# arkworks-rs/algebra

Hardware: AMD Instinct MI355X
Metric: G1 scalar-muls/sec (MSM, 2^24) (higher is better)
Workload: dtype u32

## Files before the change

### algebra_amd/_lib.py

```python
import ctypes as C
import os

_HERE = os.path.dirname(os.path.abspath(__file__))
LIB_PATH = os.environ.get("ARK_HIP_LIB") or os.path.join(_HERE, "libark_hip.so")

u64p = C.POINTER(C.c_uint64)


class ArkHipError(RuntimeError):
    def __init__(self, code, what):
        super().__init__("%s failed with code %d" % (what, code))
        self.code = code


class Radix2DomainStruct(C.Structure):
    _fields_ = [
        ("size", C.c_uint64),
        ("log_size_of_group", C.c_uint32),
        ("_pad", C.c_uint32),
        ("size_as_field_element", C.c_uint64 * 4),
        ("size_inv", C.c_uint64 * 4),
        ("group_gen", C.c_uint64 * 4),
        ("group_gen_inv", C.c_uint64 * 4),
        ("offset", C.c_uint64 * 4),
# ... 129 lines not shown
    "ark_hip_test_basefield_op": (C.c_int, [C.c_int, C.c_int, C.c_void_p, C.c_void_p, C.c_void_p, C.c_size_t]),
    "ark_hip_test_host_basefield_op": (C.c_int, [C.c_int, C.c_int, C.c_void_p, C.c_void_p, C.c_void_p, C.c_size_t]),
    "ark_hip_test_host_sw_check": (C.c_int, [C.c_int, C.c_void_p, C.c_size_t, C.c_int, C.c_int, C.c_void_p]),
    "ark_hip_test_host_sw_decompress": (C.c_int, [C.c_int, C.c_void_p, C.c_size_t, C.c_int, C.c_int, C.c_void_p, C.c_void_p]),
    "ark_hip_test_host_sw_compress": (C.c_int, [C.c_int, C.c_void_p, C.c_size_t, C.c_void_p]),
    "ark_hip_test_host_sw_mul": (C.c_int, [C.c_int, C.c_void_p, C.c_int, C.c_void_p, C.c_size_t, C.c_int, C.c_int, C.c_size_t, C.c_void_p]),
    "ark_hip_test_host_sw_add": (C.c_int, [C.c_int, C.c_void_p, C.c_void_p, C.c_int, C.c_size_t, C.c_void_p]),
    "ark_hip_test_host_sw_fold": (C.c_int, [C.c_int, C.c_void_p, C.c_void_p, C.c_int, C.c_void_p, C.c_void_p, C.c_int, C.c_int, C.c_size_t,
                                            C.c_void_p]),
    "ark_hip_test_coord_sqrt": (C.c_int, [C.c_int, C.c_void_p, C.c_void_p, C.c_void_p, C.c_size_t]),
    "ark_hip_test_host_coord_sqrt": (C.c_int, [C.c_int, C.c_void_p, C.c_void_p, C.c_void_p, C.c_size_t]),
    "ark_hip_test_point_op": (C.c_int, [C.c_int, C.c_int, C.c_void_p, C.c_void_p, C.c_void_p, C.c_size_t]),
    "ark_hip_test_msm_sharded_emulated": (C.c_int, [C.c_int, C.c_int, C.POINTER(C.c_void_p), C.POINTER(C.c_void_p),
                                                    C.POINTER(C.c_size_t), C.c_int, C.c_void_p, C.POINTER(C.c_int)]),
    "ark_hip_test_base_hash": (C.c_int, [C.c_void_p, C.c_size_t, C.POINTER(C.c_uint64)]),
    "ark_hip_test_lazy_raw_op": (C.c_int, [C.c_int, C.c_int, C.c_int, C.c_int, C.c_void_p, C.c_void_p, C.c_size_t]),
    "ark_hip_test_lazy_acc_op": (C.c_int, [C.c_int, C.c_int, C.c_void_p, C.c_void_p, C.c_void_p, C.c_size_t]),
    "ark_hip_test_relaxed_raw_op": (C.c_int, [C.c_int, C.c_int, C.c_void_p, C.c_void_p, C.c_size_t]),
    "ark_hip_test_relaxed_acc_op": (C.c_int, [C.c_int, C.c_int, C.c_void_p, C.c_void_p, C.c_void_p, C.c_size_t]),
    "ark_hip_test_msm_host_fold": (C.c_int, [C.c_int, C.c_void_p, C.c_int, C.c_int, C.c_int, C.c_void_p, C.c_void_p]),
    "ark_hip_test_msm_reduce_geometry": (C.c_int, [C.c_int, C.c_int, C.c_int, C.c_int, C.c_int, C.c_size_t, C.POINTER(C.c_uint32)]),
    "ark_hip_test_msm_sort_geometry": (C.c_int, [C.c_int, C.c_size_t, C.c_int, C.c_int, C.c_int, C.c_int, C.POINTER(C.c_int32),
                                                 C.POINTER(C.c_uint64)]),
    "ark_hip_test_msm_sort_stages": (C.c_int, [C.c_int, C.c_void_p, C.c_int, C.c_size_t, C.c_int, C.c_int, C.c_int,
                                               C.POINTER(C.c_int32), C.POINTER(C.c_uint64), C.POINTER(C.c_void_p),
                                               C.POINTER(C.c_size_t)]),
    "ark_hip_test_msm_pieces": (C.c_int, [C.c_int, C.c_void_p, C.c_void_p, C.c_int, C.c_size_t, C.c_int, C.POINTER(C.c_size_t), C.c_int,
                                          C.POINTER(C.c_int32), C.POINTER(C.c_uint64), C.c_void_p, C.c_size_t, C.c_void_p, C.c_size_t,
                                          C.c_void_p]),
    "ark_hip_test_msm_host_fold_l0": (C.c_int, [C.c_int, C.c_void_p, C.c_int, C.c_int, C.c_int, C.c_void_p, C.c_void_p]),
}
TEST_LIB_PATH = os.path.join(_HERE, "libark_hip_test.so")

_lib = None
_test_lib = None


def lib():
    global _lib
    if _lib is None:
        if not os.path.exists(LIB_PATH):
            raise ImportError(
                "algebra_amd: %s not found -- the HIP extension is not built and there is no CPU fallback "
                "(run `make -C algebra_amd/csrc -j8` or __graft_entry__.build())" % LIB_PATH)
        try:
            import torch
# ... 40 lines not shown
```

### algebra_amd/csrc/msm.cuh

```cuda
#pragma once
#include <hip/hip_runtime.h>
#include <stdio.h>
#include <stdlib.h>
#include <vector>
#include <mutex>
#include <atomic>
#include "hostpool.hpp"
#include <math.h>
#include "curves.cuh"
#include "ec28.cuh"
#include "lazyk.cuh"
#include "msm_sort.cuh"
#include "msm_plan.hpp"

namespace arkhip {

#define ARK_HIP_TRY(expr)                                                                          \
  do {                                                                                             \
    hipError_t _e = (expr);                                                                        \
    if (_e != hipSuccess) {                                                                        \
      fprintf(stderr, "ark_hip: %s failed: %s (%s:%d)\n", #expr, hipGetErrorString(_e), __FILE__, __LINE__); \
      return -(int)_e - 1000;                                                                      \
    }                                                                                              \
  } while (0)
// ... 161 lines not shown
template <class SP>
void msm_sample_widths_host(const void* h_scalars, size_t n, int mont, MsmWidths* out) {
  typedef Fp<SP> S;
  *out = MsmWidths{};
  out->max_bits = (u32)SP::BITS;
  if (n == 0) return;
  const size_t stride = n > 1024 ? n / 1024 : 1;
  size_t seen = 0;
  u32 cnt[MSM_WIDTH_CLASSES] = {0};
  for (size_t i = 0; i < n; i += stride) {
    u32 v[S::N + 1];
    (void)msm_scalar_magnitude<SP>((const u32*)h_scalars, (u32)i, mont, v, nullptr);
    u32 b = 0;
    for (int k = 0; k < S::N; k++)
      if (v[k]) b = 32u * (u32)k + 32u - (u32)__builtin_clz(v[k]);
    int cls = 0;
    for (int k = 1; k < MSM_WIDTH_CLASSES; k++) cls += b > (u32)MSM_WIDTH_TOP[k - 1] ? 1 : 0;
    cnt[cls]++;
    seen++;
  }
  for (int k = 0; k < MSM_WIDTH_CLASSES; k++) out->count[k] = (u32)((double)cnt[k] * (double)n / (double)seen);
}

template <class SP>
__global__ void __launch_bounds__(256) msm_digits_kernel(const u32* __restrict__ scalars, u32 n, int mont, int c,
                                                         int W, int narrow, u32* __restrict__ keys,
                                                         u32* __restrict__ err) {
  u32 i = blockIdx.x * blockDim.x + threadIdx.x;
  if (i >= n) return;
  typedef Fp<SP> S;
  u32 v[S::N + 1];
  const u32 flip = msm_scalar_magnitude<SP>(scalars, i, mont, v, err);
  u32 carry = 0;
  for (int w = 0; w < W; w++) {
    const int cw = msm_window_width(w, c, W, narrow);
    const u32 mask = (1u << cw) - 1u;
    const u32 half = 1u << (cw - 1);
    u32 raw = (v[0] & mask) + carry;
#pragma unroll
    for (int k = 0; k < S::N; k++) v[k] = (v[k] >> cw) | (v[k + 1] << (32 - cw));
    u32 key = KEY_NONE;
    if (w < W - 1) {
      carry = raw >= half ? 1u : 0u;
    } else {
      carry = 0;
    }
    int d = (int)raw - (int)(carry << cw);
    if (d != 0) {
      u32 mag = d < 0 ? (u32)(-d) : (u32)d;
      if (mag > half) {
        atomicOr(err, 1u);
        mag = half;
      }
      u32 sign = (d < 0 ? 0x80000000u : 0u) ^ flip;
      key = sign | (mag - 1);
    }
    keys[(size_t)w * n + i] = key;
  }
}

template <int BYTES>
__global__ void __launch_bounds__(256) msm_digits_small_kernel(const unsigned char* __restrict__ scalars, u32 n, int c, int W,
                                                               int narrow, u64 vmask, u32* __restrict__ keys) {
  u32 i = blockIdx.x * blockDim.x + threadIdx.x;
  if (i >= n) return;
  u64 v;
  if constexpr (BYTES == 1) v = scalars[i];
  else if constexpr (BYTES == 2) v = ((const unsigned short*)scalars)[i];
  else if constexpr (BYTES == 4) v = ((const u32*)scalars)[i];
  else v = ((const u64*)scalars)[i];
  v &= vmask;
  u32 carry = 0;
  for (int w = 0; w < W; w++) {
    const int cw = msm_window_width(w, c, W, narrow);
    const u32 mask = (1u << cw) - 1u;
    const u32 half = 1u << (cw - 1);
    const u32 raw = ((u32)v & mask) + carry;
    v >>= cw;
    carry = (w < W - 1 && raw >= half) ? 1u : 0u;
    const int d = (int)raw - (int)(carry << cw);
    u32 key = KEY_NONE;
// ... 927 lines not shown
    const bool fail =
        (compacted && (cscal.ensure(n * 32) || cidx.ensure(n * 4))) ||
        keys.ensure(W * n * 4) || sorted.ensure(W * n * 4) || part.ensure(W * n * 8) ||
        thist.ensure(sg.nthist * 4) || toff.ensure((sg.nthist + 2) * 4) ||
        offsets.ensure((pl.nb + 2) * 4) || sums.ensure(2 * sg.nsums * 4) ||
        order.ensure(nbk * 4) || ohist.ensure((sg.nohist + ORDER_BINS) * 4) || ooff.ensure((sg.nohist + ORDER_BINS + 2) * 4) ||
        (own_buckets && buckets.ensure(nbk * B)) ||
        lvlS[0].ensure(rg.m * Wr * B) || lvlA[0].ensure(rg.m * Wr * B) || lvlS[1].ensure(rg.npart * B) ||
        (rg.nchunks > 1 && lvlA[1].ensure(rg.npairs * B)) || (rg.two_digit && lvlA[1].ensure(Wr * rg.nsum2 * B)) ||
        hctr.ensure(64) || hlist.ensure((hg.max_heavy + 1) * sizeof(HeavyEntry)) || hitems.ensure((hg.max_items + 1) * 8) ||
        hpart.ensure((hg.max_items + 1) * B) || (pl.shared && hfinal.ensure(hg.max_heavy * B)) ||
        (sg.big_on && big.ensure(2 * sg.big_region * 4)) || (run_parts > 1 && parts.ensure(2 * (size_t)run_parts * pl.nb * B));
    return fail ? -3 : 0;
  }
  int launch_resources(bool need_side) {
    if (need_side) {
      if (!side) ARK_HIP_TRY(hipStreamCreateWithFlags(&side, hipStreamNonBlocking));
      for (auto& e : grp_ev)
        if (!e) ARK_HIP_TRY(hipEventCreateWithFlags(&e, hipEventDisableTiming));
    }
    if (!attr_set) {
      ARK_HIP_TRY(hipFuncSetAttribute((const void*)msm_part_scatter_kernel, hipFuncAttributeMaxDynamicSharedMemorySize,
                                      (int)PART_SCATTER_LDS_MAX));
      ARK_HIP_TRY(hipFuncSetAttribute((const void*)msm_part_finish_kernel, hipFuncAttributeMaxDynamicSharedMemorySize,
                                      160 * 1024 - 64));
      attr_set = true;
    }
    return 0;
  }
  void release() {
    if (probe_host) (void)hipHostFree(probe_host);
    probe_host = nullptr;
    hctr.release(); hlist.release(); hitems.release(); hpart.release(); hfinal.release();
    nzcnt.release(); cscal.release(); cidx.release();
    keys.release(); part.release(); thist.release(); toff.release(); sorted.release();
    offsets.release(); sums.release();
    order.release(); ohist.release(); ooff.release(); probe.release(); big.release(); parts.release();
    buckets.release();
    if (side) { (void)hipStreamSynchronize(side); (void)hipStreamDestroy(side); side = nullptr; }
    for (auto& e : grp_ev) { if (e) (void)hipEventDestroy(e); e = nullptr; }
    for (int i = 0; i < 2; i++) { lvlS[i].release(); lvlA[i].release(); }
    for (auto& j : jobs) {
      if (j.pinned) (void)hipHostFree(j.pinned);
      j.pinned = nullptr;
      j.pinned_cap = 0;
      if (j.done) (void)hipEventDestroy(j.done);
      if (j.acc_done) (void)hipEventDestroy(j.acc_done);
// ... 99 lines not shown
template <class C>
struct MsmCall {
  typedef XYZZ<typename C::F> Pt;
  MsmWorkspace& ws;
  MsmJob& job;
  hipStream_t stream;
  bool timing;
  const void* d_points;
  size_t wstride;
  const void* d_scalars;
  size_t n;
  int scalars_mont;
  const MsmPiece* piece;
  MsmPlan pl;
  MsmSortGeom sg;
  MsmReduceGeom rg;
  MsmHeavyGeom hg;
  int ngroups;
  bool heavy_side, lazy, compacted;
  u32 run_parts;
  int split_level;
  char* d_buckets;
  int accum;

  struct Group {
    int w0, Wg;
    size_t slot0, nslots, nbk_g;
    u32 *keys, *sorted, *offsets, *thist, *toff, *order, *sums, *ohist, *ooff, *hctr;
    u32* big;
    u32* big_count;
    uint2* part;
    HeavyEntry* hlist;
    uint2* hitems;
    char *hpart, *buckets, *parts;
    size_t max_heavy;
  } grp[2];

  void make_groups() {
    const int W = pl.W, Bbits = pl.c - 1;
    const size_t nbk = pl.nbuckets();
    const int W0 = ngroups == 2 ? (W + 1) / 2 : W;
    for (int g = 0; g < ngroups; g++) {
      Group& G = grp[g];
      G.w0 = g == 0 ? 0 : W0;
      G.Wg = g == 0 ? W0 : W - W0;
      G.slot0 = (size_t)G.w0 << Bbits;
// ... 23 lines not shown
      G.parts = run_parts > 1 ? (char*)ws.parts.p + (size_t)g * run_parts * pl.nb * Pt::BYTES : nullptr;
    }
  }

  void compact(const void* d_scalars_all, size_t n_all, const MsmProbe& pr) {
    u32* const cnt = (u32*)ws.nzcnt.p;
    u32* const off = cnt + pr.nz_blocks + 1;
    scan_exclusive(cnt, pr.nz_blocks, nullptr, off, stream);
    hipLaunchKernelGGL((msm_compact_scalars_kernel<typename C::S>), dim3(pr.nz_blocks), dim3(1024), 0, stream,
                       (const u32*)d_scalars_all, (u32)n_all, scalars_mont, pr.nz_chunk, (const u32*)off, (u32*)ws.hctr.p + 3,
                       (u32*)ws.cscal.p, (u32*)ws.cidx.p, (u32)n);
  }

  void digits(int sbytes, int sbits) {
    const int c = pl.c, W = pl.W;
    u32* const keys = (u32*)ws.keys.p;
    const u32 nblk = (u32)((n + 255) / 256);
    if (sbytes) {
      const u64 vmask = sbits >= 64 ? ~0ull : ((1ull << sbits) - 1ull);
      const unsigned char* sp = (const unsigned char*)d_scalars;
      const auto kernel = sbytes == 1 ? msm_digits_small_kernel<1> : sbytes == 2 ? msm_digits_small_kernel<2>
                          : sbytes == 4 ? msm_digits_small_kernel<4> : msm_digits_small_kernel<8>;
      hipLaunchKernelGGL(kernel, dim3(nblk), dim3(256), 0, stream, sp, (u32)n, c, W, pl.narrow, vmask, keys);
    } else {
      hipLaunchKernelGGL((msm_digits_kernel<typename C::S>), dim3(nblk), dim3(256), 0, stream, (const u32*)d_scalars,
                         (u32)n, scalars_mont, c, W, pl.narrow, keys, (u32*)ws.hctr.p + 3);
    }
  }

  int sort_group(const Group& G, hipStream_t st, bool mark) {
    const int HB = sg.HB, LB = sg.LB;
    const u32 ntiles = sg.ntiles;
    const size_t mwin = (size_t)1 << (pl.c - 1);
    const u32 nsuper_g = (u32)G.Wg << HB;
    const size_t nthist_g = (size_t)nsuper_g * ntiles;
    hipLaunchKernelGGL(msm_part_hist_kernel, dim3(ntiles, G.Wg), dim3(256), (size_t)4 << HB, st, G.keys, (u32)n, HB, LB,
                       ntiles, sg.tile, G.thist);
    scan_exclusive(G.thist, nthist_g, G.sums, G.toff, st);
    if (mark && timing) ARK_HIP_TRY(hipEventRecord(job.ev[2], st));
    hipLaunchKernelGGL(msm_part_scatter_kernel, dim3(ntiles, G.Wg), dim3(1024), sg.lds_a, st, G.keys, (u32)n, HB, LB, ntiles,
                       sg.tile, G.toff, G.part, compacted ? (const u32*)ws.cidx.p : (const u32*)nullptr);
    hipLaunchKernelGGL(msm_part_finish_kernel, dim3(nsuper_g), dim3(1024), sg.lds_b, st, G.part, G.toff, ntiles, LB, nsuper_g,
                       sg.stage_cap, sg.big_on ? PART_BIG : 0u, G.big_count, G.big, G.offsets, G.sorted);
    if (sg.big_on) {
      u32* const bigcnt = G.big + nsuper_g;
      u32* const cursor = bigcnt + G.nslots;
      hipLaunchKernelGGL(msm_part_big_hist_kernel, dim3(PART_BIG_SLICES, PART_BIG_GRID_Y), dim3(1024), (size_t)4 << LB, st,
                         G.part, G.toff, ntiles, LB, G.big_count, G.big, bigcnt);
      hipLaunchKernelGGL(msm_part_big_place_kernel, dim3(PART_BIG_SLICES, PART_BIG_GRID_Y), dim3(1024),
                         ((size_t)8 << LB) + 4096, st, G.part, G.toff, ntiles, LB, G.big_count, G.big, bigcnt, cursor, G.offsets,
                         G.sorted);
    }
    int shift = 0;
    while ((hg.mean_load >> shift) >= 64) shift++;
    const u32 noblk_g = (u32)((G.nbk_g + ORDER_TILE - 1) / ORDER_TILE);
    const int wsum = pl.shared ? pl.W : 1;
    hipLaunchKernelGGL(msm_order_hist_kernel, dim3(noblk_g), dim3(256), 0, st, G.offsets, G.nbk_g, shift, noblk_g, wsum, mwin,
                       G.ohist);
    scan_exclusive(G.ohist, (size_t)noblk_g * ORDER_BINS, G.sums, G.ooff, st);
    hipLaunchKernelGGL(msm_order_scatter_kernel, dim3(noblk_g), dim3(256), 0, st, G.offsets, G.nbk_g, shift, noblk_g, wsum, mwin,
                       G.ooff, G.order);
    return 0;
  }

  int front(const void* d_scalars_all, size_t n_all, const MsmProbe& pr, int sbytes, int sbits) {
    if (timing) ARK_HIP_TRY(hipEventRecord(job.ev[0], stream));
// ... 113 lines not shown
      job.short_job = (double)n * (double)pl.W <= 6.0e6;
      job.Q = rg.Q;
      job.d_sums = d_sums;
    }
    job.busy = true;
    return 0;
  }
};

template <class C>
struct MsmSetup {
  MsmProbe pr;
  MsmPlan pl;
  size_t n_all, n;
  bool compacted;
  MsmSortGeom sg;
  MsmReduceGeom rg;
  MsmHeavyGeom hg;
  bool lazy;
  u32 run_parts;
  int ngroups;
  bool heavy_side;
  int split_level;
  MsmCall<C> call(MsmWorkspace& ws, MsmJob& job, hipStream_t stream, bool timing, const void* d_points, size_t wstride,
                  const void* d_scalars, int scalars_mont, const MsmPiece* piece, char* d_buckets) const {
    MsmCall<C> c{ws, job, stream, timing, d_points, wstride, compacted ? ws.cscal.p : d_scalars, n, scalars_mont, piece,
                 pl, sg, rg, hg, ngroups, heavy_side, lazy, compacted, run_parts, split_level,
                 d_buckets, (piece && !piece->first) ? 1 : 0};
    c.make_groups();
    return c;
  }
};
template <class C>
int msm_setup(MsmWorkspace& ws, const void* d_scalars, size_t n, int scalars_mont, hipStream_t stream, int sbytes, int sbits,
              const MsmPlan*& prepared, size_t& wstride, const MsmPiece* piece, const MsmKnobs& knobs, MsmSetup<C>& su) {
  MsmProbe& pr = su.pr;
  if (!sbytes && !piece && n >= ((size_t)1 << 19))
    if (int rc = msm_probe_widths<C>(ws, d_scalars, n, scalars_mont, stream, knobs, prepared, wstride, pr)) return rc;
  const MsmPlan pl = prepared ? *prepared
                     : piece  ? *piece->plan
                     : pr.have_widths ? msm_plan_for_widths(C::ID, n, pr.widths, knobs)
                                      : msm_default_plan(C::ID, n, sbytes ? sbits + 1 : C::S::BITS, false, nullptr, knobs);
  const size_t n_all = n, zeros = pr.widths.count[0];
  const bool compacted = pr.measured_exact && knobs.compact && zeros * 4 >= n && zeros < n && zeros * (size_t)pl.W >= 3 * n;
  if (compacted) n = n_all - zeros;
  if ((size_t)n * (size_t)pl.W >= (1ull << 32)) return -2;
  if (prepared && (wstride < n || (size_t)pl.W * wstride >= (1ull << 31))) return -2;

  su.pl = pl;
  su.n_all = n_all;
  su.n = n;
  su.compacted = compacted;
  su.sg = msm_sort_geometry(n, pl, knobs);
  if (su.sg.lds_a > PART_SCATTER_LDS_MAX) return -2;
  su.rg = msm_reduce_geometry(pl, C::FA::LANES, C::S::BITS, C::FA::LANES == 1 ? msm_resident_lanes<C>() : 0, knobs);
  su.hg = msm_heavy_geometry(n, pl, knobs);
  su.lazy = knobs.lazy;
  su.run_parts = (su.lazy && !piece && !pl.shared) ? msm_run_parts(n, pl, pr.have_widths ? &pr.widths : nullptr, knobs) : 1u;
  su.ngroups = msm_window_groups(n, pl, piece != nullptr, knobs);
  su.heavy_side = knobs.heavy_side && su.ngroups == 1 && !piece && n >= ((size_t)1 << 20);
  su.split_level = knobs.split_level;
  return 0;
}

template <class C>
int msm_enqueue(MsmWorkspace& ws, const void* d_points, size_t wstride, const MsmPlan* prepared, const void* d_scalars,
                size_t n, int scalars_mont, hipStream_t stream, bool timing, int sbytes = 0, int sbits = 0,
                const MsmPiece* piece = nullptr, const MsmKnobs* knobs_in = nullptr) {
  typedef XYZZ<typename C::F> Pt;
  std::lock_guard<std::mutex> lock(ws.mu);
  int slot = -1;
  for (int i = 0; i < MSM_JOBS; i++)
    if (!ws.jobs[i].busy) { slot = i; break; }
  if (slot < 0) return -6;
  MsmJob& job = ws.jobs[slot];
  job.empty = (n == 0);
  job.timing = false;
  job.no_result = false;
  if (piece && (prepared || n == 0)) return -1;
  if (n == 0) {
    job.busy = true;
    return slot;
  }
  if (n >= (1ull << 31)) return -2;
// ... 313 lines not shown
```

### algebra_amd/csrc/msm_plan.hpp

```cpp
#pragma once
#include <math.h>
#include <stddef.h>
#include <stdint.h>
#include <stdio.h>
#include <stdlib.h>
#include "params.hpp"

#if defined(__HIP__)
#define ARK_PLAN_HD __host__ __device__ __forceinline__
#else
#define ARK_PLAN_HD inline
#endif

namespace arkhip {
typedef uint32_t u32;

struct MsmKnobs {
  bool lazy = true;
  bool probe = true;
  bool compact = true;
  bool heavy_side = true;
  bool big_slices = true;
  bool plan_debug = false;
  int groups = 0;
  int split_level = -1;
  size_t parts_lanes = 262144;
  int c = 0;
  int c_prepared = 0;
  int l0 = 0;
  int stage2 = -1;
  int chunk = 0;
  int heavy = 0;
  int hb = -1;
  int tile = 0;
  int run_parts = 0;
};

inline MsmKnobs msm_knobs() {
  const auto first_char = [](const char* name) { const char* e = getenv(name); return e ? e[0] : '\0'; };
  const auto number = [](const char* name, long unset) { const char* e = getenv(name); return e ? atol(e) : unset; };
  const auto within = [](long v, long lo, long hi) { return v >= lo && v <= hi ? (int)v : 0; };
  static const MsmKnobs once = [&] {
    MsmKnobs k;
    k.lazy = first_char("ARK_HIP_MSM_LAZY") != '0';
    k.probe = number("ARK_HIP_MSM_PROBE", 1) != 0;
    k.compact = first_char("ARK_HIP_MSM_COMPACT") != '0';
    k.heavy_side = number("ARK_HIP_MSM_HEAVY_SIDE", 1) != 0;
    k.big_slices = number("ARK_HIP_MSM_BIG_SLICES", 1) != 0;
    k.plan_debug = getenv("ARK_HIP_PLAN_DEBUG") != nullptr;
    k.groups = (int)number("ARK_HIP_MSM_GROUPS", 0);
    k.split_level = (int)number("ARK_HIP_MSM_SPLIT_LEVEL", -1);
    k.parts_lanes = (size_t)number("ARK_HIP_MSM_PARTS_LANES", 262144);
    return k;
  }();
  MsmKnobs k = once;
  k.c = within(number("ARK_HIP_MSM_C", 0), 3, 26);
  k.c_prepared = within(number("ARK_HIP_MSM_C_PREPARED", 0), 3, 26);
  k.l0 = within(number("ARK_HIP_MSM_L0", 0), 1, 128);
  const char s2 = first_char("ARK_HIP_MSM_STAGE2");
  k.stage2 = s2 == '0' ? 0 : (s2 == '1' ? 1 : -1);
  const long chunk = number("ARK_HIP_MSM_CHUNK", 0);
  k.chunk = (chunk & (chunk - 1)) == 0 ? within(chunk, 256, 16384) : 0;
  k.heavy = within(number("ARK_HIP_MSM_HEAVY", 0), 64, 0x7fffffff);
  k.hb = (int)number("ARK_HIP_MSM_HB", -1);
  k.tile = (int)number("ARK_HIP_MSM_TILE", 0);
  const long rp = number("ARK_HIP_MSM_RUN_PARTS", 0);
  k.run_parts = (rp & (rp - 1)) == 0 ? within(rp, 1, 8) : 0;
  return k;
}

static constexpr int MSM_WIDTH_CLASSES = 9;
static constexpr int MSM_WIDTH_TOP[MSM_WIDTH_CLASSES] = {0, 1, 8, 16, 32, 64, 128, 192, 256};
struct MsmWidths {
  u32 max_bits;
  u32 count[MSM_WIDTH_CLASSES];
// ... 145 lines not shown
  p.nb = (size_t)p.W << (best_c - 1);
  return p;
}

static inline MsmPlan msm_default_plan(int curve_id, size_t n, int bits, bool shared, const MsmWidths* widths,
                                       const MsmKnobs& knobs = msm_knobs(), bool streamed = false) {
  return msm_make_plan(n, bits, msm_mul_cost(curve_id), shared, widths, !shared && !streamed && knobs.lazy, knobs);
}

static inline MsmPlan msm_plan_for_widths(int curve_id, size_t n, const MsmWidths& w, const MsmKnobs& knobs = msm_knobs()) {
  const int slack = 8, field_bits = msm_scalar_bits(curve_id);
  int bits = field_bits;
  if ((int)w.max_bits + 1 + slack <= field_bits) bits = (w.max_bits ? (int)w.max_bits : 1) + 1;
  return msm_default_plan(curve_id, n, bits, false, &w, knobs);
}

static constexpr int PART_LO_BITS = 10;
static constexpr int PART_LO_BITS_MAX = 12;
static constexpr u32 PART_LDS_WORDS = (160 * 1024 - 64) / 4;
static constexpr int PART_TILE = 8192;
static constexpr int PART_TILE_BIG = 16384;
static constexpr size_t PART_SCATTER_LDS_MAX = 160 * 1024 - 4096 - 64;
static constexpr u32 PART_BIG = 1u << 17;
static constexpr int SCAN_TILE = 2048;
static constexpr int ORDER_TILE = 2048;
static constexpr int ORDER_BINS = 256;

static inline void msm_part_split(size_t n, int B, int* HB, int* LB, const MsmKnobs& knobs) {
  int hb = 0;
  if (B > PART_LO_BITS) {
    hb = B - PART_LO_BITS;
    if (hb > 9) {
      hb = B - PART_LO_BITS_MAX;
      if (hb < 9) hb = 9;
    }
    int lg = 0;
    while (((size_t)1 << lg) < n) lg++;
    if (hb < lg - 15) hb = lg - 15;
    if (hb > B) hb = B;
    const int v = knobs.hb;
    if (v >= 0 && v <= B && B - v <= PART_LO_BITS_MAX) hb = v;
  } else {
    int lg = 0;
    while (((size_t)1 << lg) < n) lg++;
    hb = lg - 15;
    if (hb < 0) hb = 0;
    if (hb > B) hb = B;
  }
  *HB = hb;
  *LB = B - hb;
}
static inline u32 msm_part_stage_cap(int LB) { return PART_LDS_WORDS - 1024u - (1u << LB) - 16u; }
static inline u32 msm_part_tile(int HB, const MsmKnobs& knobs) {
  const bool fits = ((size_t)8 << HB) + (size_t)PART_TILE_BIG * 8 <= PART_SCATTER_LDS_MAX;
  if (knobs.tile == PART_TILE || (knobs.tile == PART_TILE_BIG && fits)) return (u32)knobs.tile;
  return (HB >= 11 && fits) ? (u32)PART_TILE_BIG : (u32)PART_TILE;
}

struct MsmSortGeom {
  int HB, LB;
  u32 nsuper;
  u32 tile, ntiles;
  size_t nthist;
  size_t lds_a, lds_b;
  u32 stage_cap;
  bool big_on;
  size_t big_region;
  u32 noblk;
  size_t nohist, nsums;
};
static inline MsmSortGeom msm_sort_geometry(size_t n, const MsmPlan& pl, const MsmKnobs& knobs) {
  MsmSortGeom g;
  msm_part_split(n, pl.c - 1, &g.HB, &g.LB, knobs);
  g.nsuper = (u32)pl.W << g.HB;
  g.tile = msm_part_tile(g.HB, knobs);
  g.ntiles = (u32)((n + g.tile - 1) / g.tile);
  g.nthist = (size_t)g.nsuper * g.ntiles;
  g.lds_a = ((size_t)8 << g.HB) + (size_t)g.tile * 8;
  g.stage_cap = msm_part_stage_cap(g.LB);
  g.lds_b = ((size_t)(1 << g.LB) + 1024 + g.stage_cap) * 4;
  g.big_on = knobs.big_slices && n > (size_t)2 * PART_BIG;
  g.big_region = (size_t)g.nsuper + 2 * pl.nb;
  const u32 ntscan = (u32)((g.nthist + SCAN_TILE - 1) / SCAN_TILE);
  g.noblk = (u32)((pl.nbuckets() + ORDER_TILE - 1) / ORDER_TILE);
  g.nohist = (size_t)g.noblk * ORDER_BINS;
  const u32 noscan = (u32)((g.nohist + SCAN_TILE - 1) / SCAN_TILE);
  g.nsums = (size_t)(ntscan > noscan ? ntscan : noscan) + 2;
  return g;
}

struct MsmReduceGeom {
  u32 red_narrow, red_full;
  u32 L0;
  size_t m, mn;
  int nbits;
  u32 Q;
  bool two_digit;
  u32 d2, rows2;
  size_t nsum2;
  u32 chunk, nchunks;
  size_t npart, npairs;
};
// ... 74 lines not shown

static inline u32 msm_run_parts(size_t n, const MsmPlan& pl, const MsmWidths* widths, const MsmKnobs& knobs) {
  u32 run_parts = 1;
  double expect = (double)n * pl.W;
  if (widths) {
    expect = 0.0;
    for (int k = 1; k < MSM_WIDTH_CLASSES; k++) {
      int need = (MSM_WIDTH_TOP[k] + 1 + pl.c - 1) / pl.c;
      expect += (double)widths->count[k] * (need > pl.W ? pl.W : need);
    }
  }
  const double mean_run = expect / (double)pl.nb;
  while (run_parts < 8 && pl.nb * (size_t)(2 * run_parts) <= knobs.parts_lanes && mean_run >= 32.0 * (2 * run_parts)) run_parts *= 2;
  if (pl.parts) run_parts = pl.parts;
  if (knobs.run_parts) run_parts = (u32)knobs.run_parts;
  return run_parts;
}

static inline int msm_window_groups(size_t n, const MsmPlan& pl, bool piece, const MsmKnobs& knobs) {
  if (pl.shared || piece || pl.W < 6 || n < ((size_t)1 << 19)) return 1;
  return (knobs.groups == 2 || (knobs.groups != 1 && n >= ((size_t)1 << 25))) ? 2 : 1;
}

}
```

### algebra_amd/csrc/msm_sort.cuh

```cuda
#pragma once
#include <hip/hip_runtime.h>
#include <stdlib.h>
#include "fp.cuh"
#include "msm_plan.hpp"

namespace arkhip {

static constexpr u32 PART_KEY_NONE = 0xffffffffu;
static constexpr int PART_MLP = 8;
static constexpr int PART_OUT_MLP = 4;
static constexpr int PART_SCATTER_KEYS = PART_TILE_BIG / 1024;

__host__ __device__ __forceinline__ u32 msm_slot_to_bucket(u32 slot, int HB, int LB) {
  const u32 B = (u32)(HB + LB);
  const u32 w = slot >> B;
  const u32 in = slot & ((1u << B) - 1u);
  const u32 low = in >> LB;
  const u32 high = in & ((1u << LB) - 1u);
  return (w << B) | (high << HB) | low;
}

static __device__ __forceinline__ u32 part_tile_of_block(u32 b, u32 ntiles) {
  const u32 per = ntiles >> 3;
  return b < (per << 3) ? (b & 7u) * per + (b >> 3) : b;
// ... 109 lines not shown
      if (j < total) {
        const u32 bkt = e[b].x & 0x7fffffffu;
        part[dst[b]] = make_uint2((bkt >> HB) | (e[b].x & 0x80000000u), e[b].y);
      }
    }
  }
}

__device__ __forceinline__ u32 lds_inc_leading(u32* cnt, u32 key) {
  const u32 k0 = __builtin_amdgcn_readfirstlane(key);
  const unsigned long long same = __ballot(key == k0);
  u32 pos;
  if (key == k0) {
    const u32 rank = __builtin_amdgcn_mbcnt_hi((u32)(same >> 32), __builtin_amdgcn_mbcnt_lo((u32)same, 0u));
    u32 base = 0;
    if (rank == 0) base = atomicAdd(&cnt[k0], (u32)__popcll(same));
    pos = __builtin_amdgcn_readfirstlane(base) + rank;
  } else {
    pos = atomicAdd(&cnt[key], 1u);
  }
  return pos;
}

static __global__ void __launch_bounds__(1024) msm_part_finish_kernel(const uint2* __restrict__ part,
                                                                      const u32* __restrict__ tile_off, u32 ntiles,
                                                                      int LB, u32 nsuper, u32 stage_cap, u32 big_thresh,
                                                                      u32* __restrict__ big_count, u32* __restrict__ big,
                                                                      u32* __restrict__ offsets,
                                                                      u32* __restrict__ sorted) {
  extern __shared__ u32 part_lds[];
  const u32 nlow = 1u << LB;
  u32* cnt = part_lds;
  u32* wsum = part_lds + nlow;
  u32* stage = wsum + 1024;
  const u32 sb = blockIdx.x;
  const u32 start = tile_off[(size_t)sb * ntiles];
  const u32 end = tile_off[(size_t)(sb + 1) * ntiles];
  if (sb == nsuper - 1 && threadIdx.x == 0) offsets[(size_t)nsuper << LB] = end;
  if (big_thresh && end - start > big_thresh) {
    if (threadIdx.x == 0) big[atomicAdd(big_count, 1u)] = sb;
    u32* const bigcnt = big + nsuper + ((size_t)sb << LB);
    u32* const cursor = bigcnt + ((size_t)nsuper << LB);
    for (u32 b = threadIdx.x; b < nlow; b += blockDim.x) {
      bigcnt[b] = 0;
      cursor[b] = 0;
    }
    return;
  }
  for (u32 b = threadIdx.x; b < nlow; b += blockDim.x) cnt[b] = 0;
  __syncthreads();
  const u32 lmask = nlow - 1u;
  for (u32 c0 = start; c0 < end; c0 += blockDim.x * PART_MLP) {
    u32 kx[PART_MLP];
#pragma unroll
    for (int b = 0; b < PART_MLP; b++) {
      const u32 j = c0 + (u32)b * blockDim.x + threadIdx.x;
      kx[b] = j < end ? part[j].x : PART_KEY_NONE;
    }
#pragma unroll
    for (int b = 0; b < PART_MLP; b++)
      if (kx[b] != PART_KEY_NONE) lds_inc_leading(cnt, kx[b] & lmask);
  }
  __syncthreads();
  const u32 per = nlow > blockDim.x ? nlow / blockDim.x : 1u;
  const u32 b0 = threadIdx.x * per;
  u32 v = 0;
  if (b0 < nlow)
    for (u32 k = 0; k < per; k++) v += cnt[b0 + k];
  wsum[threadIdx.x] = v;
  __syncthreads();
  for (u32 o = 1; o < blockDim.x; o <<= 1) {
    u32 y = threadIdx.x >= o ? wsum[threadIdx.x - o] : 0;
    __syncthreads();
    wsum[threadIdx.x] += y;
    __syncthreads();
  }
  if (b0 < nlow) {
    u32 run = wsum[threadIdx.x] - v;
    for (u32 k = 0; k < per; k++) {
      const u32 c = cnt[b0 + k];
      cnt[b0 + k] = run;
      offsets[((size_t)sb << LB) + b0 + k] = start + run;
      run += c;
    }
  }
  __syncthreads();
  const u32 total = end - start;
  if (total <= stage_cap) {
    for (u32 c0 = start; c0 < end; c0 += blockDim.x * PART_MLP) {
      uint2 e[PART_MLP];
#pragma unroll
      for (int b = 0; b < PART_MLP; b++) {
        const u32 j = c0 + (u32)b * blockDim.x + threadIdx.x;
        e[b] = j < end ? part[j] : make_uint2(PART_KEY_NONE, 0u);
      }
#pragma unroll
      for (int b = 0; b < PART_MLP; b++) {
        if (e[b].x != PART_KEY_NONE) {
          const u32 pos = lds_inc_leading(cnt, e[b].x & lmask);
          stage[pos] = e[b].y | (e[b].x & 0x80000000u);
        }
      }
    }
    __syncthreads();
    for (u32 j = threadIdx.x; j < total; j += blockDim.x) sorted[start + j] = stage[j];
  } else {
    for (u32 j = start + threadIdx.x; j < end; j += blockDim.x) {
      uint2 e = part[j];
      u32 pos = lds_inc_leading(cnt, e.x & lmask);
      sorted[start + pos] = e.y | (e.x & 0x80000000u);
    }
// ... 131 lines not shown
```

### include/ark_hip.h

```cpp
#ifndef ARK_HIP_H
#define ARK_HIP_H
#include <stddef.h>
#include <stdint.h>
#ifdef __cplusplus
extern "C" {
#endif
#if defined(__GNUC__) || defined(__clang__)
#pragma GCC visibility push(default)
#endif

enum { ARK_HIP_BN254_FQ = 0, ARK_HIP_BN254_FR = 1, ARK_HIP_BLS12_381_FQ = 2, ARK_HIP_BLS12_381_FR = 3,
       ARK_HIP_BLS12_377_FQ = 4, ARK_HIP_BLS12_377_FR = 5 };
enum { ARK_HIP_BN254_G1 = 0, ARK_HIP_BLS12_381_G1 = 1, ARK_HIP_BLS12_377_G1 = 2, ARK_HIP_BLS12_377_G2 = 3,
       ARK_HIP_BLS12_381_G2 = 4 };
enum { ARK_HIP_OK = 0, ARK_HIP_ERR_ARG = -1, ARK_HIP_ERR_SIZE = -2, ARK_HIP_ERR_NOMEM = -3,
       ARK_HIP_ERR_SCALAR_RANGE = -4, ARK_HIP_ERR_NO_DEVICE = -5, ARK_HIP_ERR_BUSY = -6,
       ARK_HIP_ERR_COMM = -7   };

int ark_hip_device_count(void);
int ark_hip_init(int device);
int ark_hip_set_device(int device);
int ark_hip_get_device(void);
void ark_hip_shutdown(void);
int ark_hip_synchronize(void);
// ... 173 lines not shown
int ark_hip_test_field_op(int field, int op, const uint64_t* a, const uint64_t* b, uint64_t* r, size_t n);
int ark_hip_test_basefield_op(int curve, int op, const uint64_t* a, const uint64_t* b, uint64_t* r, size_t n);
int ark_hip_test_host_basefield_op(int curve, int op, const uint64_t* a, const uint64_t* b, uint64_t* r, size_t n);
int ark_hip_test_host_sw_check(int curve, const uint64_t* bases_xy, size_t n, int checks, int method, uint8_t* status);
int ark_hip_test_host_sw_decompress(int curve, const uint8_t* bytes, size_t n, int validate, int method, uint64_t* points_xy, uint8_t* status);
int ark_hip_test_host_sw_compress(int curve, const uint64_t* points_xy, size_t n, uint8_t* bytes);
int ark_hip_test_host_sw_mul(int curve, const uint64_t* points, int form, const uint64_t* scalars, size_t n_scalars,
                             int scalars_are_montgomery, int impl, size_t n, uint64_t* out_xyz);
int ark_hip_test_host_sw_add(int curve, const uint64_t* a_xyz, const uint64_t* b_xyz, int negate_b, size_t n, uint64_t* out_xyz);
int ark_hip_test_host_sw_fold(int curve, const uint64_t* lo, const uint64_t* hi, int form, const uint64_t a[4], const uint64_t b[4],
                              int scalars_are_montgomery, int impl, size_t n, uint64_t* out_xyz);
int ark_hip_test_coord_sqrt(int curve, const uint64_t* in, uint64_t* out, uint8_t* ok, size_t n);
int ark_hip_test_host_coord_sqrt(int curve, const uint64_t* in, uint64_t* out, uint8_t* ok, size_t n);
int ark_hip_test_point_op(int curve, int kind, const uint64_t* acc, const uint64_t* other, uint64_t* out, size_t n);
int ark_hip_test_msm_sharded_emulated(int curve, int world, const void* const* d_bases, const void* const* d_scalars,
                                      const size_t* n_local, int scalars_are_montgomery, uint64_t* out_xyz, int* path);
int ark_hip_test_base_hash(const uint64_t* p, size_t words, uint64_t out[2]);
int ark_hip_test_msm_host_fold(int curve, const uint64_t* parts, int windows, int nbits, int log2_l0, const int* widths,
                               uint64_t* out_xyz);
int ark_hip_test_msm_host_fold_l0(int curve, const uint64_t* parts, int windows, int nbits, int l0, const int* widths,
                                  uint64_t* out_xyz);
int ark_hip_test_msm_reduce_geometry(int curve, int c, int W, int narrow, int shared, size_t resident_lanes, uint32_t out[12]);
int ark_hip_test_msm_sort_geometry(int curve, size_t n, int c, int W, int narrow, int shared, const int32_t knobs[8], uint64_t out[32]);
int ark_hip_test_msm_sort_stages(int curve, const void* scalars, int on_device, size_t n, int mont, int sbytes, int sbits,
                                 const int32_t knobs[8], uint64_t header[32], void* const* out, const size_t* cap_words);
int ark_hip_test_msm_pieces(int curve, const void* bases, const void* scalars, int on_device, size_t n, int mont, const size_t* sizes,
                            int npieces, const int32_t knobs[12], uint64_t header[80], uint32_t* hctr_out, size_t hctr_cap_words,
                            void* buckets_out, size_t buckets_cap_bytes, uint64_t* out_xyz);
int ark_hip_test_lazy_raw_op(int field, int op, int k, int h, const uint32_t* in, uint32_t* out, size_t n);
int ark_hip_test_lazy_acc_op(int curve, int kind, const void* acc, const void* other, void* out, size_t n);
int ark_hip_test_relaxed_raw_op(int field, int op, const uint32_t* in, uint32_t* out, size_t n);
int ark_hip_test_relaxed_acc_op(int curve, int kind, const void* acc, const void* other, void* out, size_t n);

#endif

#if defined(__GNUC__) || defined(__clang__)
#pragma GCC visibility pop
#endif
#ifdef __cplusplus
}
#endif
#endif
```

Before: 470.2 million.

## Fuse digit histogram into recoding kernel and single-pass partition finish

Scalar recoding now optionally builds per-tile digit histograms in LDS as it emits keys, so the separate histogram pass over the keys can be skipped for the windows it covers. The partition finish kernel also gains a templated path that loads small slices into registers once, ranks them and scatters them from those registers, instead of reading the partition array twice. Both save global memory traffic in the sort front end. The cost is LDS atomics in the recode kernel, a 1024-thread launch shape, and higher register pressure in the finish kernel.

```diff
diff --git a/algebra_amd/_lib.py b/algebra_amd/_lib.py
--- a/algebra_amd/_lib.py
+++ b/algebra_amd/_lib.py
@@ -175,6 +175,8 @@
     "ark_hip_test_msm_reduce_geometry": (C.c_int, [C.c_int, C.c_int, C.c_int, C.c_int, C.c_int, C.c_size_t, C.POINTER(C.c_uint32)]),
     "ark_hip_test_msm_sort_geometry": (C.c_int, [C.c_int, C.c_size_t, C.c_int, C.c_int, C.c_int, C.c_int, C.POINTER(C.c_int32),
                                                  C.POINTER(C.c_uint64)]),
+    "ark_hip_test_msm_front_end": (C.c_int, [C.c_int, C.c_size_t, C.c_int, C.c_int, C.c_int, C.c_int, C.POINTER(C.c_int32),
+                                             C.POINTER(C.c_uint64)]),
     "ark_hip_test_msm_sort_stages": (C.c_int, [C.c_int, C.c_void_p, C.c_int, C.c_size_t, C.c_int, C.c_int, C.c_int,
                                                C.POINTER(C.c_int32), C.POINTER(C.c_uint64), C.POINTER(C.c_void_p),
                                                C.POINTER(C.c_size_t)]),
diff --git a/algebra_amd/csrc/msm.cuh b/algebra_amd/csrc/msm.cuh
--- a/algebra_amd/csrc/msm.cuh
+++ b/algebra_amd/csrc/msm.cuh
@@ -207,12 +207,9 @@
   for (int k = 0; k < MSM_WIDTH_CLASSES; k++) out->count[k] = (u32)((double)cnt[k] * (double)n / (double)seen);
 }
 
-template <class SP>
-__global__ void __launch_bounds__(256) msm_digits_kernel(const u32* __restrict__ scalars, u32 n, int mont, int c,
-                                                         int W, int narrow, u32* __restrict__ keys,
-                                                         u32* __restrict__ err) {
-  u32 i = blockIdx.x * blockDim.x + threadIdx.x;
-  if (i >= n) return;
+template <class SP, class OnKey>
+__device__ __forceinline__ void msm_recode_scalar(const u32* __restrict__ scalars, u32 n, u32 i, int mont, int c, int W, int narrow,
+                                                  u32* __restrict__ keys, u32* __restrict__ err, OnKey on_key) {
   typedef Fp<SP> S;
   u32 v[S::N + 1];
   const u32 flip = msm_scalar_magnitude<SP>(scalars, i, mont, v, err);
@@ -239,9 +236,39 @@
       }
       u32 sign = (d < 0 ? 0x80000000u : 0u) ^ flip;
       key = sign | (mag - 1);
+      on_key(w, key);
     }
     keys[(size_t)w * n + i] = key;
   }
+}
+
+template <class SP>
+__global__ void __launch_bounds__(256) msm_digits_kernel(const u32* __restrict__ scalars, u32 n, int mont, int c,
+                                                         int W, int narrow, u32* __restrict__ keys,
+                                                         u32* __restrict__ err) {
+  u32 i = blockIdx.x * blockDim.x + threadIdx.x;
+  if (i >= n) return;
+  msm_recode_scalar<SP>(scalars, n, i, mont, c, W, narrow, keys, err, [](int, u32) {});
+}
+
+template <class SP>
+__global__ void __launch_bounds__(1024) msm_digits_hist_kernel(const u32* __restrict__ scalars, u32 n, int mont, int c, int W,
+                                                               int narrow, u32* __restrict__ keys, u32* __restrict__ err,
+                                                               int HB, int Wh, u32 ntiles, u32 tile, u32* __restrict__ tile_hist) {
+  extern __shared__ u32 digit_lds[];
+  const u32 ncnt = (u32)Wh << HB;
+  const u32 hmask = (1u << HB) - 1u;
+  for (u32 b = threadIdx.x; b < ncnt; b += blockDim.x) digit_lds[b] = 0;
+  __syncthreads();
+  const u32 tile_id = part_tile_of_block(blockIdx.x, ntiles);
+  const u32 lo = tile_id * tile;
+  const u32 hi = lo + tile < n ? lo + tile : n;
+  for (u32 i = lo + threadIdx.x; i < hi; i += blockDim.x)
+    msm_recode_scalar<SP>(scalars, n, i, mont, c, W, narrow, keys, err, [&](int w, u32 key) {
+      if (w < Wh) atomicAdd(&digit_lds[((u32)w << HB) | (key & hmask)], 1u);
+    });
+  __syncthreads();
+  for (u32 b = threadIdx.x; b < ncnt; b += blockDim.x) tile_hist[(size_t)b * ntiles + tile_id] = digit_lds[b];
 }
 
 template <int BYTES>
@@ -1215,7 +1242,9 @@
     if (!attr_set) {
       ARK_HIP_TRY(hipFuncSetAttribute((const void*)msm_part_scatter_kernel, hipFuncAttributeMaxDynamicSharedMemorySize,
                                       (int)PART_SCATTER_LDS_MAX));
-      ARK_HIP_TRY(hipFuncSetAttribute((const void*)msm_part_finish_kernel, hipFuncAttributeMaxDynamicSharedMemorySize,
+      ARK_HIP_TRY(hipFuncSetAttribute((const void*)msm_part_finish_kernel<false>, hipFuncAttributeMaxDynamicSharedMemorySize,
+                                      160 * 1024 - 64));
+      ARK_HIP_TRY(hipFuncSetAttribute((const void*)msm_part_finish_kernel<true>, hipFuncAttributeMaxDynamicSharedMemorySize,
                                       160 * 1024 - 64));
       attr_set = true;
     }
@@ -1361,6 +1390,7 @@
   int split_level;
   char* d_buckets;
   int accum;
+  int hist_windows;
 
   struct Group {
     int w0, Wg;
@@ -1430,6 +1460,10 @@
       const auto kernel = sbytes == 1 ? msm_digits_small_kernel<1> : sbytes == 2 ? msm_digits_small_kernel<2>
                           : sbytes == 4 ? msm_digits_small_kernel<4> : msm_digits_small_kernel<8>;
       hipLaunchKernelGGL(kernel, dim3(nblk), dim3(256), 0, stream, sp, (u32)n, c, W, pl.narrow, vmask, keys);
+    } else if (hist_windows) {
+      hipLaunchKernelGGL((msm_digits_hist_kernel<typename C::S>), dim3(sg.ntiles), dim3(1024), ((size_t)hist_windows << sg.HB) * 4,
+                         stream, (const u32*)d_scalars, (u32)n, scalars_mont, c, W, pl.narrow, keys, (u32*)ws.hctr.p + 3, sg.HB,
+                         hist_windows, sg.ntiles, sg.tile, (u32*)ws.thist.p);
     } else {
       hipLaunchKernelGGL((msm_digits_kernel<typename C::S>), dim3(nblk), dim3(256), 0, stream, (const u32*)d_scalars,
                          (u32)n, scalars_mont, c, W, pl.narrow, keys, (u32*)ws.hctr.p + 3);
@@ -1442,14 +1476,16 @@
     const size_t mwin = (size_t)1 << (pl.c - 1);
     const u32 nsuper_g = (u32)G.Wg << HB;
     const size_t nthist_g = (size_t)nsuper_g * ntiles;
-    hipLaunchKernelGGL(msm_part_hist_kernel, dim3(ntiles, G.Wg), dim3(256), (size_t)4 << HB, st, G.keys, (u32)n, HB, LB,
-                       ntiles, sg.tile, G.thist);
+    if (G.w0 + G.Wg > hist_windows)
+      hipLaunchKernelGGL(msm_part_hist_kernel, dim3(ntiles, G.Wg), dim3(256), (size_t)4 << HB, st, G.keys, (u32)n, HB, LB,
+                         ntiles, sg.tile, G.thist);
     scan_exclusive(G.thist, nthist_g, G.sums, G.toff, st);
     if (mark && timing) ARK_HIP_TRY(hipEventRecord(job.ev[2], st));
     hipLaunchKernelGGL(msm_part_scatter_kernel, dim3(ntiles, G.Wg), dim3(1024), sg.lds_a, st, G.keys, (u32)n, HB, LB, ntiles,
                        sg.tile, G.toff, G.part, compacted ? (const u32*)ws.cidx.p : (const u32*)nullptr);
-    hipLaunchKernelGGL(msm_part_finish_kernel, dim3(nsuper_g), dim3(1024), sg.lds_b, st, G.part, G.toff, ntiles, LB, nsuper_g,
-                       sg.stage_cap, sg.big_on ? PART_BIG : 0u, G.big_count, G.big, G.offsets, G.sorted);
+    hipLaunchKernelGGL(sg.keep_cap ? msm_part_finish_kernel<true> : msm_part_finish_kernel<false>, dim3(nsuper_g), dim3(1024),
+                       sg.lds_b, st, G.part, G.toff, ntiles, LB, nsuper_g, sg.stage_cap, sg.big_on ? PART_BIG : 0u, G.big_count,
+                       G.big, G.offsets, G.sorted, sg.keep_cap);
     if (sg.big_on) {
       u32* const bigcnt = G.big + nsuper_g;
       u32* const cursor = bigcnt + G.nslots;
@@ -1609,11 +1645,12 @@
   int ngroups;
   bool heavy_side;
   int split_level;
+  int hist_windows;
   MsmCall<C> call(MsmWorkspace& ws, MsmJob& job, hipStream_t stream, bool timing, const void* d_points, size_t wstride,
                   const void* d_scalars, int scalars_mont, const MsmPiece* piece, char* d_buckets) const {
     MsmCall<C> c{ws, job, stream, timing, d_points, wstride, compacted ? ws.cscal.p : d_scalars, n, scalars_mont, piece,
                  pl, sg, rg, hg, ngroups, heavy_side, lazy, compacted, run_parts, split_level,
-                 d_buckets, (piece && !piece->first) ? 1 : 0};
+                 d_buckets, (piece && !piece->first) ? 1 : 0, hist_windows};
     c.make_groups();
     return c;
   }
@@ -1647,6 +1684,7 @@
   su.ngroups = msm_window_groups(n, pl, piece != nullptr, knobs);
   su.heavy_side = knobs.heavy_side && su.ngroups == 1 && !piece && n >= ((size_t)1 << 20);
   su.split_level = knobs.split_level;
+  su.hist_windows = msm_digit_hist_windows(pl, su.sg, su.ngroups, sbytes, compacted, knobs);
   return 0;
 }
 
diff --git a/algebra_amd/csrc/msm_plan.hpp b/algebra_amd/csrc/msm_plan.hpp
--- a/algebra_amd/csrc/msm_plan.hpp
+++ b/algebra_amd/csrc/msm_plan.hpp
@@ -34,6 +34,8 @@
   int hb = -1;
   int tile = 0;
   int run_parts = 0;
+  bool digit_hist = true;
+  bool finish_once = true;
 };
 
 inline MsmKnobs msm_knobs() {
@@ -51,6 +53,8 @@
     k.groups = (int)number("ARK_HIP_MSM_GROUPS", 0);
     k.split_level = (int)number("ARK_HIP_MSM_SPLIT_LEVEL", -1);
     k.parts_lanes = (size_t)number("ARK_HIP_MSM_PARTS_LANES", 262144);
+    k.digit_hist = first_char("ARK_HIP_MSM_DIGIT_HIST") != '0';
+    k.finish_once = first_char("ARK_HIP_MSM_FINISH_ONCE") != '0';
     return k;
   }();
   MsmKnobs k = once;
@@ -242,6 +246,8 @@
 static constexpr int PART_TILE_BIG = 16384;
 static constexpr size_t PART_SCATTER_LDS_MAX = 160 * 1024 - 4096 - 64;
 static constexpr u32 PART_BIG = 1u << 17;
+static constexpr size_t DIGIT_HIST_LDS_MAX = 64 * 1024;
+static constexpr u32 PART_FINISH_KEEP = 36;
 static constexpr int SCAN_TILE = 2048;
 static constexpr int ORDER_TILE = 2048;
 static constexpr int ORDER_BINS = 256;
@@ -271,6 +277,10 @@
   *LB = B - hb;
 }
 static inline u32 msm_part_stage_cap(int LB) { return PART_LDS_WORDS - 1024u - (1u << LB) - 16u; }
+static inline u32 msm_part_keep_cap(u32 stage_cap, const MsmKnobs& knobs) {
+  const u32 keep = PART_FINISH_KEEP * 1024u;
+  return knobs.finish_once ? (stage_cap < keep ? stage_cap : keep) : 0u;
+}
 static inline u32 msm_part_tile(int HB, const MsmKnobs& knobs) {
   const bool fits = ((size_t)8 << HB) + (size_t)PART_TILE_BIG * 8 <= PART_SCATTER_LDS_MAX;
   if (knobs.tile == PART_TILE || (knobs.tile == PART_TILE_BIG && fits)) return (u32)knobs.tile;
@@ -284,6 +294,7 @@
   size_t nthist;
   size_t lds_a, lds_b;
   u32 stage_cap;
+  u32 keep_cap;
   bool big_on;
   size_t big_region;
   u32 noblk;
@@ -298,6 +309,7 @@
   g.nthist = (size_t)g.nsuper * g.ntiles;
   g.lds_a = ((size_t)8 << g.HB) + (size_t)g.tile * 8;
   g.stage_cap = msm_part_stage_cap(g.LB);
+  g.keep_cap = msm_part_keep_cap(g.stage_cap, knobs);
   g.lds_b = ((size_t)(1 << g.LB) + 1024 + g.stage_cap) * 4;
   g.big_on = knobs.big_slices && n > (size_t)2 * PART_BIG;
   g.big_region = (size_t)g.nsuper + 2 * pl.nb;
@@ -418,4 +430,13 @@
   return (knobs.groups == 2 || (knobs.groups != 1 && n >= ((size_t)1 << 25))) ? 2 : 1;
 }
 
-}
+static inline int msm_digit_hist_windows(const MsmPlan& pl, const MsmSortGeom& sg, int ngroups, int sbytes, bool compacted,
+                                         const MsmKnobs& knobs) {
+  if (!knobs.digit_hist || sbytes || compacted) return 0;
+  const auto fits = [&](int windows) { return ((size_t)windows << sg.HB) * 4 <= DIGIT_HIST_LDS_MAX; };
+  if (fits(pl.W)) return pl.W;
+  const int W0 = (pl.W + 1) / 2;
+  return ngroups == 2 && fits(W0) ? W0 : 0;
+}
+
+}
diff --git a/algebra_amd/csrc/msm_sort.cuh b/algebra_amd/csrc/msm_sort.cuh
--- a/algebra_amd/csrc/msm_sort.cuh
+++ b/algebra_amd/csrc/msm_sort.cuh
@@ -155,12 +155,13 @@
   return pos;
 }
 
+template <bool ONCE>
 static __global__ void __launch_bounds__(1024) msm_part_finish_kernel(const uint2* __restrict__ part,
                                                                       const u32* __restrict__ tile_off, u32 ntiles,
                                                                       int LB, u32 nsuper, u32 stage_cap, u32 big_thresh,
                                                                       u32* __restrict__ big_count, u32* __restrict__ big,
                                                                       u32* __restrict__ offsets,
-                                                                      u32* __restrict__ sorted) {
+                                                                      u32* __restrict__ sorted, u32 keep_cap = 0) {
   extern __shared__ u32 part_lds[];
   const u32 nlow = 1u << LB;
   u32* cnt = part_lds;
@@ -183,16 +184,40 @@
   for (u32 b = threadIdx.x; b < nlow; b += blockDim.x) cnt[b] = 0;
   __syncthreads();
   const u32 lmask = nlow - 1u;
-  for (u32 c0 = start; c0 < end; c0 += blockDim.x * PART_MLP) {
-    u32 kx[PART_MLP];
-#pragma unroll
-    for (int b = 0; b < PART_MLP; b++) {
-      const u32 j = c0 + (u32)b * blockDim.x + threadIdx.x;
-      kx[b] = j < end ? part[j].x : PART_KEY_NONE;
-    }
-#pragma unroll
-    for (int b = 0; b < PART_MLP; b++)
-      if (kx[b] != PART_KEY_NONE) lds_inc_leading(cnt, kx[b] & lmask);
+  const u32 total = end - start;
+  const bool once = ONCE && total <= keep_cap;
+  u32 kept[ONCE ? PART_FINISH_KEEP : 1], kidx[ONCE ? PART_FINISH_KEEP : 1];
+  if (once) {
+    if constexpr (ONCE) {
+#pragma unroll
+      for (u32 b = 0; b < PART_FINISH_KEEP; b++) {
+        const u32 j = b * 1024u + threadIdx.x;
+        if (j < total) {
+          const uint2 e = part[start + j];
+          kept[b] = e.x;
+          kidx[b] = e.y;
+        }
+      }
+#pragma unroll
+      for (u32 b = 0; b < PART_FINISH_KEEP; b++) {
+        if (b * 1024u + threadIdx.x < total) {
+          const u32 rank = lds_inc_leading(cnt, kept[b] & lmask);
+          kept[b] = (kept[b] & (0x80000000u | lmask)) | (rank << 12);
+        }
+      }
+    }
+  } else {
+    for (u32 c0 = start; c0 < end; c0 += blockDim.x * PART_MLP) {
+      u32 kx[PART_MLP];
+#pragma unroll
+      for (int b = 0; b < PART_MLP; b++) {
+        const u32 j = c0 + (u32)b * blockDim.x + threadIdx.x;
+        kx[b] = j < end ? part[j].x : PART_KEY_NONE;
+      }
+#pragma unroll
+      for (int b = 0; b < PART_MLP; b++)
+        if (kx[b] != PART_KEY_NONE) lds_inc_leading(cnt, kx[b] & lmask);
+    }
   }
   __syncthreads();
   const u32 per = nlow > blockDim.x ? nlow / blockDim.x : 1u;
@@ -218,8 +243,16 @@
     }
   }
   __syncthreads();
-  const u32 total = end - start;
-  if (total <= stage_cap) {
+  if (once) {
+    if constexpr (ONCE) {
+#pragma unroll
+      for (u32 b = 0; b < PART_FINISH_KEEP; b++)
+        if (b * 1024u + threadIdx.x < total)
+          stage[cnt[kept[b] & lmask] + ((kept[b] >> 12) & 0xffffu)] = kidx[b] | (kept[b] & 0x80000000u);
+    }
+    __syncthreads();
+    for (u32 j = threadIdx.x; j < total; j += blockDim.x) sorted[start + j] = stage[j];
+  } else if (total <= stage_cap) {
     for (u32 c0 = start; c0 < end; c0 += blockDim.x * PART_MLP) {
       uint2 e[PART_MLP];
 #pragma unroll
diff --git a/include/ark_hip.h b/include/ark_hip.h
--- a/include/ark_hip.h
+++ b/include/ark_hip.h
@@ -219,6 +219,7 @@
                                   uint64_t* out_xyz);
 int ark_hip_test_msm_reduce_geometry(int curve, int c, int W, int narrow, int shared, size_t resident_lanes, uint32_t out[12]);
 int ark_hip_test_msm_sort_geometry(int curve, size_t n, int c, int W, int narrow, int shared, const int32_t knobs[8], uint64_t out[32]);
+int ark_hip_test_msm_front_end(int curve, size_t n, int c, int sbytes, int sbits, int compacted, const int32_t* knobs, uint64_t out[8]);
 int ark_hip_test_msm_sort_stages(int curve, const void* scalars, int on_device, size_t n, int mont, int sbytes, int sbits,
                                  const int32_t knobs[8], uint64_t header[32], void* const* out, const size_t* cap_words);
 int ark_hip_test_msm_pieces(int curve, const void* bases, const void* scalars, int on_device, size_t n, int mont, const size_t* sizes,
```

After: 472.3 million (median of 6 runs). No clear change (+0.4%).
